# TheIllusionistMirage/libKPEG

Hardware: NVIDIA B200
Metric: decode_mpixel_per_s (higher is better)
Workload: dtype u8/int16 entropy decode, f32 IDCT (f64 on the exact path)

## Files before the change

### libkpeg_b200/csrc/k2_expand.cu

```cuda
#include <cuda_runtime.h>
#include <stddef.h>
#include <stdint.h>

#include "entropy_core.h"
#include "kernels.cuh"
#include "kpeg_common.h"

namespace kpeg {

#ifndef KPEG_EXPAND_BATCH
#define KPEG_EXPAND_BATCH 16
#endif
constexpr int EXPAND_BATCH = KPEG_EXPAND_BATCH;
#ifndef KPEG_EXPAND_MIN_CTAS
#define KPEG_EXPAND_MIN_CTAS 12
#endif
constexpr int EXPAND_THREADS = 128;
#ifndef KPEG_EXPAND_PREFETCH_AHEAD
#define KPEG_EXPAND_PREFETCH_AHEAD 0
#endif
constexpr uint32_t EXPAND_PREFETCH_AHEAD = KPEG_EXPAND_PREFETCH_AHEAD;
constexpr uint32_t EXPAND_PREFETCH_LINES = 112;
constexpr uint32_t BIAS2 = COEF_BIAS | (COEF_BIAS << 16);

__device__ __forceinline__ void st_shared_u16(uint32_t addr, uint32_t v)
{
    asm volatile("st.shared.u16 [%0], %1;" ::"r"(addr), "h"((uint16_t)v) : "memory");
}

template <int NC>
struct ExpandSmem {
    static constexpr int NB = IDCT_MCUS_PER_CTA * NC;
    uint4 coef[NB * 8];
    int32_t carry[4];
    uint32_t reset_slot;
    uint32_t mi0;
};

template <int NC>
__global__ void __launch_bounds__(EXPAND_THREADS, KPEG_EXPAND_MIN_CTAS) expand_kernel(ExpandArgs a)
{
    constexpr int NM = IDCT_MCUS_PER_CTA;
    constexpr int NB = NM * NC;
    constexpr int NW = EXPAND_THREADS / 32;
    constexpr uint32_t TILE_SLOTS = NB * 64u;
    __shared__ __align__(128) ExpandSmem<NC> sm;

    const int t = threadIdx.x;
    const uint32_t warp = (uint32_t)t >> 5, lane = (uint32_t)t & 31u;
    const uint32_t strip = blockIdx.x;
    const uint32_t mcu0 = strip * NM, blk0 = mcu0 * NC;
    const uint32_t total_mcus = a.g.nimages * a.g.mcus_per_image;
    const uint32_t s0 = blk0 * 64u;

    const uint32_t nsub = a.meta->nsub;
    const uint32_t first0 = min(__ldg(a.strip_sub + strip), nsub - 1u);
    if (EXPAND_PREFETCH_AHEAD != 0u && strip + EXPAND_PREFETCH_AHEAD < a.nstrips) {
        const uint32_t fs = min(__ldg(a.strip_sub + strip + EXPAND_PREFETCH_AHEAD), nsub - 1u);
        const char *g0 = reinterpret_cast<const char *>(a.rec + ((size_t)(fs >> 5) * a.rec_kmax) * 32u);
        const uint32_t lines = min(a.rec_kmax, EXPAND_PREFETCH_LINES);
        for (uint32_t k = (uint32_t)t; k < 2u * lines; k += EXPAND_THREADS) {
            const uint32_t grp = k >= lines ? 1u : 0u;
            asm volatile("prefetch.global.L2 [%0];" ::"l"(g0 + ((size_t)grp * a.rec_kmax + (k - grp * lines)) * 128u));
        }
    }
    for (int i = t; i < NB * 8; i += EXPAND_THREADS)
        sm.coef[i] = make_uint4(BIAS2, BIAS2, BIAS2, BIAS2);
    if (t == 0) {
        const uint32_t img = mcu0 / a.g.mcus_per_image, mi = mcu0 - img * a.g.mcus_per_image;
        sm.mi0 = mi;
        const uint32_t mreset = a.g.restart_interval ? mi - mi % a.g.restart_interval : 0u;
        sm.reset_slot = (img * a.g.mcus_per_image + mreset) * (uint32_t)NC * 64u;
        sm.carry[0] = sm.carry[1] = sm.carry[2] = 0;
    }
    __syncthreads();
    const uint32_t tile_addr = (uint32_t)__cvta_generic_to_shared(sm.coef);

    const bool pair = a.g.sub_bits >= 1024u;
    const uint32_t per_chunk = pair ? 16u : 32u, half = pair ? lane >> 4 : 0u, kstep = pair ? 2u : 1u;
    uint32_t first = first0;
    for (int chunk = 0; chunk < 256; ++chunk, first += per_chunk) {
        const uint32_t sub = first + (pair ? lane & 15u : lane);
        bool act = sub < nsub;
        const uint32_t ss = act ? __ldg(a.start_slot + sub) : 0xFFFFFFFFu;
        const uint32_t nr = act ? __ldg(a.nrec + sub) : 0u;
        act = act && (ss <= s0 || ss - s0 < TILE_SLOTS);
        uint32_t n = 0, stride = 128u;
        const uint32_t *base = a.rec;
        if (act) {
            n = min(nr & 1023u, a.rec_kmax);
            if (nr >> 10) {
                base = a.rec_alt + (size_t)((nr >> 10) - 1u) * a.rec_kmax;
                stride = 4u;
            } else {
                base = a.rec + ((size_t)(sub >> 5) * a.rec_kmax) * 32u + (sub & 31u);
            }
        }
        const uint32_t off0 = act ? (ss & ~63u) - s0 : TILE_SLOTS;
        const uint32_t mine = pair ? (n + 1u - half) >> 1 : n;
        const uint32_t nmax = __reduce_max_sync(0xffffffffu, mine);
        const size_t rstride = (size_t)stride * kstep;
        const char *bp = reinterpret_cast<const char *>(base) + (size_t)half * stride + (size_t)(warp * EXPAND_BATCH) * rstride;
        const size_t step = (size_t)(NW * EXPAND_BATCH) * rstride;
        for (uint32_t k0 = warp * EXPAND_BATCH; k0 < nmax; k0 += NW * EXPAND_BATCH, bp += step) {
            uint32_t r[EXPAND_BATCH];
#pragma unroll
            for (int u = 0; u < EXPAND_BATCH; ++u)
                r[u] = k0 + (uint32_t)u < mine ? __ldg(reinterpret_cast<const uint32_t *>(bp + (size_t)u * rstride)) : 0xFFFFFFFFu;
#pragma unroll
            for (int u = 0; u < EXPAND_BATCH; ++u) {
                const uint32_t off = off0 + record_pos(r[u]);
                if (off < TILE_SLOTS)
                    st_shared_u16(tile_addr + coef_tile_byte(off), r[u]);
            }
        }
        if (!__shfl_sync(0xffffffffu, act && sub + 1u < nsub ? 1 : 0, 31))
            break;
    }
    if (warp == NW - 1) {
        const uint32_t ss = __ldg(a.start_slot + first0);
        const uint32_t reset_slot = sm.reset_slot;
        int part[3] = {0, 0, 0};
        if (ss < s0 && reset_slot < s0) {
            const uint32_t nr = __ldg(a.nrec + first0);
            const uint32_t n = min(nr & 1023u, a.rec_kmax);
            const uint32_t *base = (nr >> 10) ? a.rec_alt + (size_t)((nr >> 10) - 1u) * a.rec_kmax
                                              : a.rec + ((size_t)(first0 >> 5) * a.rec_kmax) * 32u + (first0 & 31u);
            const uint32_t stride = (nr >> 10) ? 1u : 32u;
            const uint32_t entry = ss & ~63u;
            for (uint32_t k = lane; k < n; k += 32u) {
                const uint32_t r = __ldg(base + (size_t)k * stride);
                const uint32_t at = entry + record_pos(r);
                if ((at & 63u) == 0u && at < s0 && at >= reset_slot) {
                    const uint32_t c = NC == 3 ? (at >> 6) % 3u : 0u;
                    const int v = record_value(r);
                    part[0] += c == 0u ? v : 0;
                    part[1] += c == 1u ? v : 0;
                    part[2] += c == 2u ? v : 0;
                }
            }
        }
#pragma unroll
        for (int c = 0; c < 3; ++c)
            part[c] = __reduce_add_sync(0xffffffffu, part[c]);
        if (lane == 0) {
            int pre[3] = {0, 0, 0};
            if (ss > reset_slot && reset_slot < s0)
                dcs_unpack(a.dcpre[first0], pre);
            sm.carry[0] = pre[0] + part[0];
            sm.carry[1] = pre[1] + part[1];
            sm.carry[2] = pre[2] + part[2];
        }
    }
    __syncthreads();

    if (t < NB) {
        const uint32_t comp = warp, ml = lane;
        const uint32_t bl = ml * NC + comp;
        const bool active = mcu0 + ml < total_mcus;
        const uint32_t dc_addr = tile_addr + bl * 128u + ((bl & 7u) << 4);
        const uint32_t dcw = sm.coef[bl * 8u + (bl & 7u)].x;
        const int dcdiff = active ? (int)(dcw & 0xFFFFu) - (int)COEF_BIAS : 0;
        bool reset = false;
        if (active) {
            uint32_t mi = sm.mi0 + ml;
            if (mi >= a.g.mcus_per_image)
                mi %= a.g.mcus_per_image;
            reset = a.g.restart_interval ? (mi % a.g.restart_interval) == 0u : mi == 0u;
        }
        int v = dcdiff;
        uint32_t f = reset ? 1u : 0u;
#pragma unroll
        for (int d = 1; d < 32; d <<= 1) {
            const int ov = __shfl_up_sync(0xffffffffu, v, d);
            const uint32_t of = __shfl_up_sync(0xffffffffu, f, d);
            if ((int)ml >= d) {
                v = f ? v : v + ov;
                f |= of;
            }
        }
        const int dcv = (int)(short)(v + (f ? 0 : sm.carry[comp]));
        if (active) {
            if ((a.g.flags & 1u) && dcdiff == 0) {
                sm.coef[bl * 8u + (bl & 7u)] = make_uint4((((uint32_t)dcv + COEF_BIAS) & 0xFFFFu) | (COEF_BIAS << 16), BIAS2, BIAS2, BIAS2);
#pragma unroll
                for (uint32_t k = 1; k < 8; ++k)
                    sm.coef[bl * 8u + (k ^ (bl & 7u))] = make_uint4(BIAS2, BIAS2, BIAS2, BIAS2);
            } else {
                st_shared_u16(dc_addr, (uint32_t)dcv + COEF_BIAS);
            }
        }
    }
    __syncthreads();

    if (t == 0) {
        asm volatile("fence.proxy.async.shared::cta;" ::: "memory");
        char *dst = reinterpret_cast<char *>(a.tiles) + (size_t)strip * (NB * 128u);
        asm volatile("cp.async.bulk.global.shared::cta.bulk_group [%0], [%1], %2;" ::"l"(dst), "r"(tile_addr), "r"((uint32_t)(NB * 128)) : "memory");
        asm volatile("cp.async.bulk.commit_group;" ::: "memory");
        asm volatile("cp.async.bulk.wait_group.read 0;" ::: "memory");
    }
}

__global__ void __launch_bounds__(256) tiles_from_matrix_kernel(JobGeom g, const int16_t *coef, const int16_t *dc, uint4 *tiles,
                                                                uint32_t padded_blocks)
{
    const uint32_t i = blockIdx.x * 256u + threadIdx.x;
    const uint32_t b = i >> 3, k = i & 7u;
    if (b >= padded_blocks)
        return;
    uint4 v = make_uint4(0, 0, 0, 0);
    if (b < g.total_blocks) {
        v = __ldg(reinterpret_cast<const uint4 *>(coef) + i);
        const int dcdiff = (int)__ldg(coef + (size_t)b * 64u);
        if ((g.flags & 1u) && dcdiff == 0)
            v = make_uint4(0, 0, 0, 0);
        if (k == 0u)
            v.x = (v.x & 0xFFFF0000u) | ((uint32_t)(uint16_t)__ldg(dc + b));
    }
    tiles[coef_tile_chunk(b, k)] = make_uint4(v.x ^ BIAS2, v.y ^ BIAS2, v.z ^ BIAS2, v.w ^ BIAS2);
}

__global__ void __launch_bounds__(256) matrix_from_tiles_kernel(const uint4 *tiles, uint4 *coef, uint32_t total_blocks)
{
    const uint32_t i = blockIdx.x * 256u + threadIdx.x;
    const uint32_t b = i >> 3, k = i & 7u;
    if (b >= total_blocks)
        return;
    const uint4 v = __ldg(tiles + coef_tile_chunk(b, k));
    coef[i] = make_uint4(v.x ^ BIAS2, v.y ^ BIAS2, v.z ^ BIAS2, v.w ^ BIAS2);
}

__global__ void __launch_bounds__(256) interleave_tiles_kernel(const uint4 *t0, const uint4 *t1, const uint4 *t2, uint4 *out,
                                                               uint32_t nmcu_padded)
{
    const uint32_t i = blockIdx.x * 256u + threadIdx.x;
    const uint32_t gb = i >> 3, k = i & 7u;
    const uint32_t m = gb / 3u, c = gb - m * 3u;
    if (m >= nmcu_padded)
        return;
    const uint4 *src = c == 0u ? t0 : (c == 1u ? t1 : t2);
    out[coef_tile_chunk(gb, k)] = __ldg(src + coef_tile_chunk(m, k));
}

void launch_interleave_tiles(const void *t0, const void *t1, const void *t2, void *out, uint32_t nmcu_padded, cudaStream_t s,
                             uint32_t *launches)
{
    const uint32_t chunks = nmcu_padded * 3u * 8u;
    interleave_tiles_kernel<<<(chunks + 255u) / 256u, 256, 0, s>>>(reinterpret_cast<const uint4 *>(t0), reinterpret_cast<const uint4 *>(t1),
                                                                   reinterpret_cast<const uint4 *>(t2), reinterpret_cast<uint4 *>(out), nmcu_padded);
    ++*launches;
}

void launch_expand(const ExpandArgs &a, cudaStream_t s, uint32_t *launches)
{
    const uint32_t total_mcus = a.g.nimages * a.g.mcus_per_image;
    const uint32_t grid = (total_mcus + IDCT_MCUS_PER_CTA - 1) / IDCT_MCUS_PER_CTA;
    if (a.g.ncomp == 3)
        expand_kernel<3><<<grid, EXPAND_THREADS, 0, s>>>(a);
    else
        expand_kernel<1><<<grid, EXPAND_THREADS, 0, s>>>(a);
    ++*launches;
}

void launch_tiles_from_matrix(const JobGeom &g, const int16_t *coef, const int16_t *dc, void *tiles, cudaStream_t s, uint32_t *launches)
{
    const uint32_t per = (uint32_t)IDCT_MCUS_PER_CTA * g.ncomp;
    const uint32_t padded = (g.total_blocks + per - 1u) / per * per;
    tiles_from_matrix_kernel<<<(padded * 8u + 255u) / 256u, 256, 0, s>>>(g, coef, dc, reinterpret_cast<uint4 *>(tiles), padded);
    ++*launches;
}

void launch_matrix_from_tiles(const void *tiles, int16_t *coef, uint32_t total_blocks, cudaStream_t s)
{
    matrix_from_tiles_kernel<<<(total_blocks * 8u + 255u) / 256u, 256, 0, s>>>(reinterpret_cast<const uint4 *>(tiles),
                                                                               reinterpret_cast<uint4 *>(coef), total_blocks);
}

}
```

Before: 86930.

## Spread DC carry scan over whole CTA, precompute reset mask, cheapen record addressing

The DC entry-carry reduction now runs across all 128 threads, with shared-memory atomics, instead of only the last warp. Thread 0 precomputes a per-MCU restart bitmask so the DC scan threads no longer do per-lane modulo arithmetic. The record load loop uses 32-bit mad.wide addressing, a signed remaining count, and an inlined swizzle address. This trades a little extra atomic and sync traffic for less serial work and cheaper per-record address math in the hot expand loop.

New measurement: 86200, median of 6. Within noise of the previous version (-0.8%).

```diff
diff --git a/libkpeg_b200/csrc/k2_expand.cu b/libkpeg_b200/csrc/k2_expand.cu
--- a/libkpeg_b200/csrc/k2_expand.cu
+++ b/libkpeg_b200/csrc/k2_expand.cu
@@ -28,14 +28,61 @@
     asm volatile("st.shared.u16 [%0], %1;" ::"r"(addr), "h"((uint16_t)v) : "memory");
 }
 
+__device__ __forceinline__ const uint32_t *record_addr(const uint32_t *p, uint32_t k, uint32_t stride_bytes)
+{
+    const uint32_t *q;
+    asm("mad.wide.u32 %0, %1, %2, %3;" : "=l"(q) : "r"(k), "r"(stride_bytes), "l"(p));
+    return q;
+}
+
 template <int NC>
 struct ExpandSmem {
     static constexpr int NB = IDCT_MCUS_PER_CTA * NC;
     uint4 coef[NB * 8];
     int32_t carry[4];
     uint32_t reset_slot;
-    uint32_t mi0;
+    uint32_t reset_mask;
 };
+
+template <int NC>
+__device__ __forceinline__ void dc_entry_carry(const ExpandArgs &a, ExpandSmem<NC> &sm, uint32_t first0, uint32_t ss, uint32_t nr,
+                                               uint32_t s0, int t)
+{
+    const uint32_t reset_slot = sm.reset_slot;
+    int part[3] = {0, 0, 0};
+    if (ss < s0 && reset_slot < s0) {
+        const uint32_t n = min(nr & 1023u, a.rec_kmax);
+        const uint32_t *base = (nr >> 10) ? a.rec_alt + (size_t)((nr >> 10) - 1u) * a.rec_kmax
+                                          : a.rec + ((size_t)(first0 >> 5) * a.rec_kmax) * 32u + (first0 & 31u);
+        const uint32_t stride = (nr >> 10) ? 1u : 32u;
+        const uint32_t entry = ss & ~63u;
+#pragma unroll 4
+        for (uint32_t k = (uint32_t)t; k < n; k += EXPAND_THREADS) {
+            const uint32_t r = __ldg(base + (size_t)k * stride);
+            const uint32_t at = entry + record_pos(r);
+            if ((at & 63u) == 0u && at < s0 && at >= reset_slot) {
+                const uint32_t c = NC == 3 ? (at >> 6) % 3u : 0u;
+                const int v = record_value(r);
+                part[0] += c == 0u ? v : 0;
+                part[1] += c == 1u ? v : 0;
+                part[2] += c == 2u ? v : 0;
+            }
+        }
+    }
+    if (t == 0 && ss > reset_slot && reset_slot < s0) {
+        int pre[3] = {0, 0, 0};
+        dcs_unpack(a.dcpre[first0], pre);
+        part[0] += pre[0];
+        part[1] += pre[1];
+        part[2] += pre[2];
+    }
+#pragma unroll
+    for (int c = 0; c < NC; ++c) {
+        const int v = __reduce_add_sync(0xffffffffu, part[c]);
+        if ((t & 31) == 0 && v != 0)
+            atomicAdd(&sm.carry[c], v);
+    }
+}
 
 template <int NC>
 __global__ void __launch_bounds__(EXPAND_THREADS, KPEG_EXPAND_MIN_CTAS) expand_kernel(ExpandArgs a)
@@ -67,14 +114,23 @@
     for (int i = t; i < NB * 8; i += EXPAND_THREADS)
         sm.coef[i] = make_uint4(BIAS2, BIAS2, BIAS2, BIAS2);
     if (t == 0) {
-        const uint32_t img = mcu0 / a.g.mcus_per_image, mi = mcu0 - img * a.g.mcus_per_image;
-        sm.mi0 = mi;
-        const uint32_t mreset = a.g.restart_interval ? mi - mi % a.g.restart_interval : 0u;
-        sm.reset_slot = (img * a.g.mcus_per_image + mreset) * (uint32_t)NC * 64u;
+        const uint32_t mpi = a.g.mcus_per_image, ri = a.g.restart_interval;
+        const uint32_t img = mcu0 / mpi, mi = mcu0 - img * mpi;
+        const uint32_t mreset = ri ? mi - mi % ri : 0u;
+        sm.reset_slot = (img * mpi + mreset) * (uint32_t)NC * 64u;
         sm.carry[0] = sm.carry[1] = sm.carry[2] = 0;
+        uint32_t mask = 0u, m = mi == mreset ? 0u : min(mpi - mi, ri ? mreset + ri - mi : mpi - mi), im = mi + m == mpi ? 0u : mi + m;
+        while (m < (uint32_t)NM) {
+            mask |= 1u << m;
+            const uint32_t step = ri ? min(ri, mpi - im) : mpi - im;
+            m += step;
+            im = im + step == mpi ? 0u : im + step;
+        }
+        sm.reset_mask = mask;
     }
     __syncthreads();
-    const uint32_t tile_addr = (uint32_t)__cvta_generic_to_shared(sm.coef);
+    uint32_t tile_addr = (uint32_t)__cvta_generic_to_shared(sm.coef);
+    asm volatile("" : "+r"(tile_addr));
 
     const bool pair = a.g.sub_bits >= 1024u;
     const uint32_t per_chunk = pair ? 16u : 32u, half = pair ? lane >> 4 : 0u, kstep = pair ? 2u : 1u;
@@ -85,73 +141,37 @@
         const uint32_t ss = act ? __ldg(a.start_slot + sub) : 0xFFFFFFFFu;
         const uint32_t nr = act ? __ldg(a.nrec + sub) : 0u;
         act = act && (ss <= s0 || ss - s0 < TILE_SLOTS);
-        uint32_t n = 0, stride = 128u;
+        const uint32_t n = act ? min(nr & 1023u, a.rec_kmax) : 0u;
+        const uint32_t mine = pair ? (n + 1u - half) >> 1 : n;
         const uint32_t *base = a.rec;
-        if (act) {
-            n = min(nr & 1023u, a.rec_kmax);
-            if (nr >> 10) {
-                base = a.rec_alt + (size_t)((nr >> 10) - 1u) * a.rec_kmax;
-                stride = 4u;
-            } else {
-                base = a.rec + ((size_t)(sub >> 5) * a.rec_kmax) * 32u + (sub & 31u);
-            }
-        }
-        const uint32_t off0 = act ? (ss & ~63u) - s0 : TILE_SLOTS;
-        const uint32_t mine = pair ? (n + 1u - half) >> 1 : n;
+        uint32_t sw = 32u;
+        if (nr >> 10) {
+            base = a.rec_alt + (size_t)((nr >> 10) - 1u) * a.rec_kmax;
+            sw = 1u;
+        } else {
+            base = a.rec + ((size_t)(sub >> 5) * a.rec_kmax) * 32u + (sub & 31u);
+        }
+        const uint32_t off0 = mine != 0u ? (ss & ~63u) - s0 : TILE_SLOTS;
         const uint32_t nmax = __reduce_max_sync(0xffffffffu, mine);
-        const size_t rstride = (size_t)stride * kstep;
-        const char *bp = reinterpret_cast<const char *>(base) + (size_t)half * stride + (size_t)(warp * EXPAND_BATCH) * rstride;
-        const size_t step = (size_t)(NW * EXPAND_BATCH) * rstride;
-        for (uint32_t k0 = warp * EXPAND_BATCH; k0 < nmax; k0 += NW * EXPAND_BATCH, bp += step) {
+        const uint32_t rs = sw * kstep, rsb = rs * 4u;
+        const uint32_t *p = base + half * sw + warp * EXPAND_BATCH * rs;
+        int left = (int)mine - (int)(warp * EXPAND_BATCH);
+        for (uint32_t k0 = warp * EXPAND_BATCH; k0 < nmax; k0 += NW * EXPAND_BATCH, p += NW * EXPAND_BATCH * rs, left -= NW * EXPAND_BATCH) {
             uint32_t r[EXPAND_BATCH];
 #pragma unroll
             for (int u = 0; u < EXPAND_BATCH; ++u)
-                r[u] = k0 + (uint32_t)u < mine ? __ldg(reinterpret_cast<const uint32_t *>(bp + (size_t)u * rstride)) : 0xFFFFFFFFu;
+                r[u] = u < left ? __ldg(record_addr(p, (uint32_t)u, rsb)) : 0xFFFFFFFFu;
 #pragma unroll
             for (int u = 0; u < EXPAND_BATCH; ++u) {
                 const uint32_t off = off0 + record_pos(r[u]);
                 if (off < TILE_SLOTS)
-                    st_shared_u16(tile_addr + coef_tile_byte(off), r[u]);
+                    st_shared_u16((tile_addr + off * 2u) ^ ((off >> 2) & 0x70u), r[u]);
             }
         }
         if (!__shfl_sync(0xffffffffu, act && sub + 1u < nsub ? 1 : 0, 31))
             break;
     }
-    if (warp == NW - 1) {
-        const uint32_t ss = __ldg(a.start_slot + first0);
-        const uint32_t reset_slot = sm.reset_slot;
-        int part[3] = {0, 0, 0};
-        if (ss < s0 && reset_slot < s0) {
-            const uint32_t nr = __ldg(a.nrec + first0);
-            const uint32_t n = min(nr & 1023u, a.rec_kmax);
-            const uint32_t *base = (nr >> 10) ? a.rec_alt + (size_t)((nr >> 10) - 1u) * a.rec_kmax
-                                              : a.rec + ((size_t)(first0 >> 5) * a.rec_kmax) * 32u + (first0 & 31u);
-            const uint32_t stride = (nr >> 10) ? 1u : 32u;
-            const uint32_t entry = ss & ~63u;
-            for (uint32_t k = lane; k < n; k += 32u) {
-                const uint32_t r = __ldg(base + (size_t)k * stride);
-                const uint32_t at = entry + record_pos(r);
-                if ((at & 63u) == 0u && at < s0 && at >= reset_slot) {
-                    const uint32_t c = NC == 3 ? (at >> 6) % 3u : 0u;
-                    const int v = record_value(r);
-                    part[0] += c == 0u ? v : 0;
-                    part[1] += c == 1u ? v : 0;
-                    part[2] += c == 2u ? v : 0;
-                }
-            }
-        }
-#pragma unroll
-        for (int c = 0; c < 3; ++c)
-            part[c] = __reduce_add_sync(0xffffffffu, part[c]);
-        if (lane == 0) {
-            int pre[3] = {0, 0, 0};
-            if (ss > reset_slot && reset_slot < s0)
-                dcs_unpack(a.dcpre[first0], pre);
-            sm.carry[0] = pre[0] + part[0];
-            sm.carry[1] = pre[1] + part[1];
-            sm.carry[2] = pre[2] + part[2];
-        }
-    }
+    dc_entry_carry<NC>(a, sm, first0, __ldg(a.start_slot + first0), __ldg(a.nrec + first0), s0, t);
     __syncthreads();
 
     if (t < NB) {
@@ -161,15 +181,8 @@
         const uint32_t dc_addr = tile_addr + bl * 128u + ((bl & 7u) << 4);
         const uint32_t dcw = sm.coef[bl * 8u + (bl & 7u)].x;
         const int dcdiff = active ? (int)(dcw & 0xFFFFu) - (int)COEF_BIAS : 0;
-        bool reset = false;
-        if (active) {
-            uint32_t mi = sm.mi0 + ml;
-            if (mi >= a.g.mcus_per_image)
-                mi %= a.g.mcus_per_image;
-            reset = a.g.restart_interval ? (mi % a.g.restart_interval) == 0u : mi == 0u;
-        }
         int v = dcdiff;
-        uint32_t f = reset ? 1u : 0u;
+        uint32_t f = (sm.reset_mask >> ml) & 1u;
 #pragma unroll
         for (int d = 1; d < 32; d <<= 1) {
             const int ov = __shfl_up_sync(0xffffffffu, v, d);
```
